# koskja/linalg-solver

Hardware: AMD Instinct MI355X
Metric: fp64_lu_gflops (higher is better)
Workload: dtype f64; 1 GPU; 8192x8192 f64 LU with partial pivoting (getrf), u11 generator, resident in HBM; n=8192, nb=128, panel_mode=4, lookahead=1, parallelism=single GPU, resident_inputs=189

## Files before the change

### linalg_solver_amd/csrc/api.hip

```cpp
#include <stdarg.h>
#include <stdlib.h>
#include <string.h>

#include <algorithm>

#include "common.h"

namespace lsx {

static thread_local char g_err[512] = "";

void set_error(const char *fmt, ...) {
    va_list ap;
    va_start(ap, fmt);
    vsnprintf(g_err, sizeof(g_err), fmt, ap);
    va_end(ap);
}

static int grow(void **p, size_t *have, size_t need) {
    if (need <= *have) return LSX_OK;
    if (*p) {
        LSX_HIP(hipFree(*p));
        *p = nullptr;
        *have = 0;
// ... 215 lines not shown
    const size_t pass_bytes = pad256(256 + (size_t)nsteps * sizeof(int)), ctr_bytes = pad256((size_t)nsteps * 8 * sizeof(int));
    const size_t col0_bytes = pad256((size_t)nsteps * 2 * sizeof(int));
    const size_t words = pass_bytes + ctr_bytes + col0_bytes + pad256((size_t)nsteps * sizeof(int));
    if (area_x == 0 || 3 * area_x + words > h->scratch_bytes) { set_error("getrf_lookahead_x: scratch"); return LSX_ERR_INTERNAL; }
    LSX_TRY(grow(&h->moves_all, &h->moves_all_bytes, (size_t)nsteps * 2048));
    JoinSide join{h, side, main_s, main_s};
    char *wbase = (char *)h->scratch + 3 * area_x;
    int *xcc_word = (int *)wbase;
    int *pass = (int *)(wbase + 256);
    int *counters = (int *)(wbase + pass_bytes);
    int *col0 = (int *)(wbase + pass_bytes + ctr_bytes);
    int *ready = (int *)(wbase + pass_bytes + ctr_bytes + col0_bytes);
    for (int s = 0; s < 3; ++s) LSX_HIP(hipMemsetAsync((char *)h->scratch + (size_t)s * area_x, 0, area_x, main_s));
    LSX_HIP(hipMemsetAsync(wbase, 0, words, main_s));
    LSX_HIP(hipMemsetD32Async((hipDeviceptr_t)xcc_word, 1, 1, main_s));
    pa.area_bytes = area_x;
    pa.xcc_word = xcc_word;
    LSX_HIP(hipEventRecord(h->ev_start, main_s));
    LSX_HIP(hipStreamWaitEvent(side, h->ev_start, 0));
    auto list = [&](int s) { return (int2 *)((char *)h->moves_all + (size_t)s * 2048); };
    T *Tinv2[2] = {Tinv, Tinv + (size_t)((nb + 63) / 64) * 4096};
    {
        OnStream g(h, side);
        pa.list = list(0);
        pa.area_off = 0;
        LSX_TRY(launch_panel<T>(h, n - k0, (n - k0) < nb ? (n - k0) : nb, A + (size_t)k0 * lda + k0, lda, k0, d_ipiv + k0, d_info, pa));
        if (!pa.listed) { set_error("getrf_lookahead_x: panel without a gather list"); return LSX_ERR_INTERNAL; }
    }
    const bool use_col0 = !h->x_events;
    bool prev_col0 = false;
    int prev_tiles = 0;
    int step = 0;
    int left_done = 0;
    for (int k = k0; k < n; k += nb, ++step) {
        const int jb = (n - k < nb) ? n - k : nb;
        const int rest = n - k - jb;
        if (rest <= 0) break;
        T *Akk = A + (size_t)k * lda + k;
        T *Ti = Tinv2[step & 1];
        T *A12 = A + (size_t)k * lda + k + jb;
        T *L21 = A + (size_t)(k + jb) * lda + k;
        T *A22 = A + (size_t)(k + jb) * lda + k + jb;
        const int jb2 = rest < nb ? rest : nb;
        bool fused_all = false;
        {
            OnStream g(h, side);
            const bool counted = step > 0 && prev_col0;
            if (step > 0 && !counted) LSX_HIP(hipStreamWaitEvent(side, h->ev_next, 0));
            const int all = launch_chain_fused<T>(h, list(step), d_info, jb, Akk, lda, Ti, jb2, A + k + jb, lda, k,
                                                  counted ? col0 + 2 * (step - 1) + 1 : nullptr, prev_tiles, ready + step);
            if (all < 0) return all;
            if (all == 1) {
                const int fused = launch_chain_head<T>(h, list(step), d_info, jb, Akk, lda, Ti, jb2, A + k + jb, lda, k,
                                                       counted ? col0 + 2 * (step - 1) + 1 : nullptr, prev_tiles);
                if (fused < 0) return fused;
                if (fused == 1) {
                    if (counted) LSX_TRY(launch_wait_count(h, col0 + 2 * (step - 1) + 1, prev_tiles, d_info));
                    LSX_TRY(launch_trtri<T>(h, 1, jb, Akk, lda, Ti));
                    LSX_TRY(launch_laswp_moves<T>(h, list(step), jb2, A + k + jb, lda, k));
                }
            }
            fused_all = all == LSX_OK;
            if (!fused_all) {
                LSX_HIP(hipEventRecord(h->ev_panel, side));
                LSX_TRY(launch_trsm_block<T>(h, 1, jb, jb2, Akk, lda, Ti, A12, lda));
            }
            LSX_TRY(launch_gemm_sub<T>(h, rest, jb2, jb, L21, lda, A12, lda, A22, lda, mfma));
        }
        if (fused_all) LSX_TRY(launch_wait_count(h, ready + step, 2, d_info));
        else LSX_HIP(hipStreamWaitEvent(main_s, h->ev_panel, 0));
        GemmDone did;
        if (rest > jb2) {
            LSX_TRY(launch_laswp_moves<T>(h, list(step), rest - jb2, A + k + jb + jb2, lda, k));
            LSX_TRY(launch_trsm_block<T>(h, 1, jb, rest - jb2, Akk, lda, Ti, A12 + jb2, lda));
            GemmPlan plan = mfma;
            plan.counters = counters + 8 * step;
            plan.avoid_word = xcc_word;
            plan.pass_word = pass + step;
            plan.col0 = use_col0 ? col0 + 2 * step : nullptr;
            LSX_TRY(launch_gemm_sub<T>(h, rest, rest - jb2, jb, L21, lda, A12 + jb2, lda, A22 + jb2, lda, plan, &did));
        }
        const bool cur_col0 = did.queued && did.col0_complete;
        LSX_HIP(hipMemsetAsync((char *)h->scratch + (size_t)(step % 3) * area_x, 0, area_x, main_s));
        LSX_HIP(hipEventRecord(h->ev_next, main_s));
        if (h->left_per_step && (rest <= 5632 || k <= 4096)) {
            if (left_done < step) {
                LSX_TRY(launch_laswp_left_all<T>(h, A, lda, k0 + left_done * nb, nb, step - left_done, list(left_done)));
                left_done = step;
            }
            if (k > 0) LSX_TRY(launch_laswp_moves<T>(h, list(step), k, A, lda, k));
            left_done = step + 1;
        }
        {
            OnStream g(h, side);
            const bool tall = (rest > 6400 && (sizeof(T) == 8 || rest <= 8192)) || rest > 12800;
            if (did.queued && (!cur_col0 || tall)) LSX_TRY(launch_gate(h, pass + step, 2 * h->num_cu / 8));
            pa.list = list(step + 1);
            pa.area_off = (size_t)((step + 1) % 3) * area_x;
            LSX_TRY(launch_panel<T>(h, rest, jb2, A22, lda, k + jb, d_ipiv + k + jb, d_info, pa));
            if (!pa.listed) { set_error("getrf_lookahead_x: panel without a gather list"); return LSX_ERR_INTERNAL; }
        }
        prev_col0 = cur_col0;
        prev_tiles = did.col0_tiles;
    }
    LSX_HIP(hipEventRecord(h->ev_panel, side));
    LSX_HIP(hipStreamWaitEvent(main_s, h->ev_panel, 0));
    join.armed = false;
    return launch_laswp_left_all<T>(h, A, lda, k0 + left_done * nb, nb, nsteps - left_done, list(left_done));
}

int ensure_getrf_workspace(lsx_handle_t h, int n, size_t elem) {
    LSX_TRY(ensure_scratch(h, pad256(16 * ((size_t)n / 32 + 2)) + 2 * pad256(elem * 2 * (size_t)n) +
                                  ((size_t)n / 32 + 2) * 5248 + 8192 +
                                  3 * panel_x_area_bytes(h, h->panel_mode, n, elem) + 16384 +
                                  ((size_t)n / 16 + 2) * 40));
    const size_t tinv_elems = (size_t)((h->nb * h->kblock + 63) / 64) * 64 * 64;
    return grow(&h->ws2, &h->ws2_bytes, 2 * pad256(tinv_elems * elem));
}

template <typename T>
static int getrf_dev(lsx_handle_t h, int n, T *A, int lda, int32_t *d_ipiv, int *d_info, bool percolumn = false) {
    LSX_ARG(n >= 0 && lda >= n && A && d_ipiv);
    if (n == 0) return LSX_OK;
    const int nb = h->nb;
    PanelArgs pa(h, h->moves_buf[0]);
    if (percolumn) pa.mode = 0;
    GemmPlan mfma;
    mfma.mfma_only = true;
    LSX_TRY(ensure_getrf_workspace(h, n, sizeof(T)));
    T *Tinv = (T *)h->ws2;
    if (!d_info) d_info = h->dev_status + 2;
    LSX_HIP(hipMemsetAsync(d_info, 0, sizeof(int), h->stream));
    int LOOKAHEAD_MIN = sizeof(T) == 8 ? 7168 : 10240;
    if (pa.mode == 4) LOOKAHEAD_MIN = sizeof(T) == 8 ? 2048 : 4096;
    if (h->lookahead_min > 0) LOOKAHEAD_MIN = h->lookahead_min;
    int k_end = n;
    if (h->lookahead && !percolumn && n >= LOOKAHEAD_MIN && h->kblock == 1) k_end = 0;
    const int W = nb * h->kblock;
    for (int k = 0; k < k_end; k += W) {
        const int w = (n - k < W) ? n - k : W;
        for (int j = 0; j < w; j += nb) {
            const int c = k + j;
            const int jb = (w - j < nb) ? w - j : nb;
            T *Acc = A + (size_t)c * lda + c;
            LSX_TRY(launch_panel<T>(h, n - c, jb, Acc, lda, c, d_ipiv + c, d_info, pa));
            if (pa.listed) {
                LSX_TRY(launch_laswp_moves_around<T>(h, (const int2 *)pa.list, n, A, lda, c, c, jb));
            } else {
                LSX_TRY(launch_laswp<T>(h, c, A, lda, c, jb, d_ipiv + c));
                LSX_TRY(launch_laswp<T>(h, n - c - jb, A + c + jb, lda, c, jb, d_ipiv + c));
            }
            const int inner = w - j - jb;
            if (inner > 0) {
                T *A12 = A + (size_t)c * lda + c + jb;
                LSX_TRY(launch_trtri<T>(h, 1, jb, Acc, lda, Tinv));
                LSX_TRY(launch_trsm_block<T>(h, 1, jb, inner, Acc, lda, Tinv, A12, lda));
                LSX_TRY(launch_gemm_sub<T>(h, n - c - jb, inner, jb, A + (size_t)(c + jb) * lda + c, lda, A12,
                                           lda, A + (size_t)(c + jb) * lda + c + jb, lda, mfma));
            }
        }
        const int rest = n - k - w;
        if (rest > 0) {
            T *Akk = A + (size_t)k * lda + k;
            T *A12 = A + (size_t)k * lda + k + w;
            LSX_TRY(launch_trtri<T>(h, 1, w, Akk, lda, Tinv));
            if (w > nb && nb % 64 == 0) {
                for (int j = 0; j < w; j += nb) {
                    const int jb = (w - j < nb) ? w - j : nb;
// ... 788 lines not shown
    return LSX_OK;
}

int lsx_synchronize(lsx_handle_t h) {
    LSX_DEVICE_GUARD(h);
    LSX_ARG(h);
    LSX_HIP(hipStreamSynchronize(h->stream));
    return LSX_OK;
}

int lsx_check_status(lsx_handle_t h) {
    LSX_ARG(h);
    LSX_DEVICE_GUARD(h);
    return check_dev_status(h);
}

int lsx_set_option(lsx_handle_t h, const char *key, int value) {
    LSX_DEVICE_GUARD(h);
    LSX_ARG(h && key);
    if (!strcmp(key, "nb")) {
        LSX_ARG(value >= 16 && value <= 128 && value % 16 == 0);
        h->nb = value;
    } else if (!strcmp(key, "panel")) {
        LSX_ARG(value >= 0 && value <= 4);
        if (value == 1 || value == 2) {
            set_error("panel modes 1 and 2 (superseded kernels) were removed: use 0, 3 or 4");
            return LSX_ERR_ARG;
        }
        h->panel_mode = value;
    } else if (!strcmp(key, "trsv")) {
        LSX_ARG(value >= 0 && value <= 2);
        h->trsv_mode = value;
    } else if (!strcmp(key, "gemm_tiles32")) {
        LSX_ARG(value == 0 || value == 1);
        h->gemm_no_tiles32 = !value;
    } else if (!strcmp(key, "gemm_queue_test")) {
        LSX_ARG(value >= 0 && value <= 3);
        h->gemm_queue_test = value;
    } else if (!strcmp(key, "gemm_stagger")) {
        LSX_ARG(value >= 0 && value <= 64);
        h->gemm_stagger = value;
    } else if (!strcmp(key, "gemm_waves")) {
        LSX_ARG(value == 0 || value == 4 || value == 8);
        h->gemm_waves = value;
    } else if (!strcmp(key, "kblock")) {
        LSX_ARG(value == 1 || value == 2);
        h->kblock = value;
    } else if (!strcmp(key, "panel_rt")) {
        LSX_ARG(value == 2 || value == 4 || value == 8);
        h->panel_rt = value;
    } else if (!strcmp(key, "panel_nt")) {
        LSX_ARG(value == 0 || value == 256 || value == 512 || value == 1024);
        h->panel_nt = value;
    } else if (!strcmp(key, "rref_blocked")) {
        LSX_ARG(value == 0 || value == 1);
        h->rref_blocked = value;
    } else if (!strcmp(key, "xrows_limit")) {
        LSX_ARG(value >= 0);
        h->xrows_limit = value;
    } else if (!strcmp(key, "getri_structured")) {
        LSX_ARG(value == 0 || value == 1);
        h->getri_plain = !value;
    } else if (!strcmp(key, "x_events")) {
        LSX_ARG(value == 0 || value == 1);
        h->x_events = value;
    } else if (!strcmp(key, "hybrid")) {
        LSX_ARG(value == 0 || value == 1);
        h->hybrid_off = !value;
    } else if (!strcmp(key, "prof_sample")) {
        LSX_ARG(value >= 1);
        h->prof.sample = value;
    } else if (!strcmp(key, "panel_spin_limit")) {
        LSX_ARG(value != 0);
        h->panel_spin_limit = value;
    } else if (!strcmp(key, "trsv_spin_limit")) {
        LSX_ARG(value >= 0);
        h->spin_limit = value;
    } else if (!strcmp(key, "getri_pairs")) {
        LSX_ARG(value == 0 || value == 1);
        h->getri_pairs = value;
    } else if (!strcmp(key, "left_per_step")) {
        LSX_ARG(value == 0 || value == 1);
        h->left_per_step = value;
    } else if (!strcmp(key, "chain_fused")) {
        LSX_ARG(value == 0 || value == 1);
        h->chain_fused = value;
    } else if (!strcmp(key, "rref_first_fast")) {
        LSX_ARG(value == 0 || value == 1);
        h->rref_first_fast = value;
    } else if (!strcmp(key, "chain_wait_limit")) {
        LSX_ARG(value >= 0);
        h->chain_wait_limit = value;
    } else if (!strcmp(key, "panel_debug")) {
        h->panel_debug = value != 0;
    } else if (!strcmp(key, "lookahead")) {
        LSX_ARG(value == 0 || value == 1);
        h->lookahead = value;
    } else if (!strcmp(key, "lookahead_min")) {
        LSX_ARG(value >= 0);
        h->lookahead_min = value;
    } else if (!strcmp(key, "getrs_t_blocked_min")) {
        LSX_ARG(value >= 0);
        h->getrs_t_blocked_min = value;
    } else {
        set_error("unknown option '%s'", key);
        return LSX_ERR_ARG;
    }
    return LSX_OK;
}

int lsx_get_option(lsx_handle_t h, const char *key, int *value) {
    LSX_DEVICE_GUARD(h);
    LSX_ARG(h && key && value);
    if (!strcmp(key, "nb")) *value = h->nb;
    else if (!strcmp(key, "panel")) *value = h->panel_mode;
    else if (!strcmp(key, "lookahead")) *value = h->lookahead;
    else if (!strcmp(key, "lookahead_min")) *value = h->lookahead_min;
    else if (!strcmp(key, "panel_rt")) *value = h->panel_rt;
    else if (!strcmp(key, "kblock")) *value = h->kblock;
    else if (!strcmp(key, "gemm_waves")) *value = h->gemm_waves;
    else if (!strcmp(key, "gemm_stagger")) *value = h->gemm_stagger;
    else if (!strcmp(key, "trsv")) *value = h->trsv_mode;
    else if (!strcmp(key, "panel_nt")) *value = h->panel_nt;
    else if (!strcmp(key, "chain_wait_limit")) *value = h->chain_wait_limit;
    else if (!strcmp(key, "rref_first_fast")) *value = h->rref_first_fast;
    else if (!strcmp(key, "chain_fused")) *value = h->chain_fused;
    else if (!strcmp(key, "left_per_step")) *value = h->left_per_step;
    else if (!strcmp(key, "getri_pairs")) *value = h->getri_pairs;
    else if (!strcmp(key, "rref_first_used")) *value = h->rref_first_used;
    else if (!strcmp(key, "panel_fallbacks")) *value = h->panel_fallbacks;
    else if (!strcmp(key, "num_cu")) *value = h->num_cu;
    else if (!strcmp(key, "gecon_solves")) *value = h->gecon_solves;
    else if (!strcmp(key, "gerfs_steps")) *value = h->gerfs_steps;
    else if (!strcmp(key, "gerfs_solves")) *value = h->gerfs_solves;
    else if (!strcmp(key, "getrs_t_blocked_min")) *value = h->getrs_t_blocked_min;
    else if (!strcmp(key, "getrs_t_path")) *value = h->getrs_t_path;
    else { set_error("unknown option '%s'", key); return LSX_ERR_ARG; }
    return LSX_OK;
}

int lsx_getrf_f64(lsx_handle_t h, int n, double *A, int lda, int32_t *ipiv, int *info) {
    LSX_DEVICE_GUARD(h);
    return getrf_host<double>(h, n, A, lda, ipiv, info);
}
int lsx_getrs_f64(lsx_handle_t h, int n, int nrhs, const double *LU, int lda, const int32_t *ipiv,
                  double *B, int ldb) {
    LSX_DEVICE_GUARD(h);
    return getrs_host<double>(h, n, nrhs, LU, lda, ipiv, B, ldb);
}
int lsx_gesv_f64(lsx_handle_t h, int n, int nrhs, const double *A, int lda, double *B, int ldb,
                 int *info, double *pivot_ratio) {
    LSX_DEVICE_GUARD(h);
    return gesv_host<double>(h, n, nrhs, A, lda, B, ldb, info, pivot_ratio);
}
int lsx_getrf_f32(lsx_handle_t h, int n, float *A, int lda, int32_t *ipiv, int *info) {
    LSX_DEVICE_GUARD(h);
    return getrf_host<float>(h, n, A, lda, ipiv, info);
}
int lsx_getrs_f32(lsx_handle_t h, int n, int nrhs, const float *LU, int lda, const int32_t *ipiv,
                  float *B, int ldb) {
    LSX_DEVICE_GUARD(h);
    return getrs_host<float>(h, n, nrhs, LU, lda, ipiv, B, ldb);
}
int lsx_gesv_f32(lsx_handle_t h, int n, int nrhs, const float *A, int lda, float *B, int ldb,
                 int *info, double *pivot_ratio) {
    LSX_DEVICE_GUARD(h);
    return gesv_host<float>(h, n, nrhs, A, lda, B, ldb, info, pivot_ratio);
}

}

namespace lsx {

template <typename T>
static int getri_host(lsx_handle_t h, int n, const T *A, int lda, T *Ainv, int ldi, int *info, double *pivot_ratio) {
    LSX_ARG(h && n >= 0 && lda >= n && ldi >= n);
    if (info) *info = 0;
    if (pivot_ratio) *pivot_ratio = 1.0;
    if (n == 0) return LSX_OK;
    LSX_ARG(A && Ainv);
    const int ld = ld_for(n);
    LSX_TRY(ensure_ws(h, 2 * pad256(sizeof(T) * (size_t)n * ld) + pad256(sizeof(int32_t) * n) + 1024));
    Carver c(h->ws);
    T *dA = c.take<T>((size_t)n * ld);
    T *dI = c.take<T>((size_t)n * ld);
    int32_t *dp = c.take<int32_t>(n);
    int *dinfo = c.take<int>(1);
    double *dprobe = c.take<double>(2);
    LSX_TRY(h2d<T>(h, n, n, A, lda, dA, ld));
    LSX_TRY(launch_amax<T>(h, n, n, dA, ld, dprobe));
    int hinfo = 0;
    LSX_TRY(factor_from_host<T>(h, n, A, lda, dA, ld, dp, dinfo, &hinfo));
    LSX_TRY(launch_diag_minabs<T>(h, n, dA, ld, dprobe));
    double probe[2] = {0, 0};
    LSX_HIP(hipMemcpyAsync(probe, dprobe, sizeof(probe), hipMemcpyDeviceToHost, h->stream));
    LSX_HIP(hipStreamSynchronize(h->stream));
    if (info) *info = hinfo;
    if (pivot_ratio) *pivot_ratio = probe[0] > 0 ? probe[1] / probe[0] : 0.0;
    if (hinfo != 0) return LSX_OK;
    LSX_TRY(getri_dev<T>(h, n, dA, ld, dp, dI, ld));
    LSX_TRY(d2h<T>(h, n, n, dI, ld, Ainv, ldi));
    LSX_HIP(hipStreamSynchronize(h->stream));
    return LSX_OK;
}

template <typename T>
static int det_host(lsx_handle_t h, int n, const T *A, int lda, double *sign, double *mant, int64_t *exp2) {
    LSX_ARG(h && n >= 0 && lda >= n && sign && mant && exp2);
    if (n == 0) { *sign = 1; *mant = 0.5; *exp2 = 1; return LSX_OK; }
    LSX_ARG(A);
// ... 672 lines not shown
```

### linalg_solver_amd/csrc/common.h

```cpp
#pragma once
#include <hip/hip_runtime.h>
#include <stdint.h>
#include <stdio.h>
#include <string>
#include <vector>

#include "../../include/lsx.h"

#ifdef LSX_TSTAMP
static __device__ long long *lsx_ts_buf;
struct TsScope {
    int id;
    __device__ void put(int tag) {
        long long *b = lsx_ts_buf;
        const int i = atomicAdd((int *)b, 1);
        if (i < (1 << 20)) { b[1 + 2 * i] = tag; b[2 + 2 * i] = wall_clock64(); }
    }
    __device__ TsScope(int id_) : id(id_) { if (lsx_ts_buf && threadIdx.x == 0 && blockIdx.x == 0 && blockIdx.y == 0) put(id); }
    __device__ ~TsScope() { if (lsx_ts_buf && threadIdx.x == 0) put(id | 0x100); }
};
#define LSX_TS(id) TsScope ts_scope_(id)
#define LSX_TS_SETTER(name) extern "C" void lsx_ts_set_##name(long long *p) { (void)hipMemcpyToSymbol(HIP_SYMBOL(lsx_ts_buf), &p, sizeof p); }
#else
#define LSX_TS(id)
#define LSX_TS_SETTER(name)
#endif

namespace lsx {

void set_error(const char *fmt, ...);

#define LSX_HIP(call)                                                                     \
    do {                                                                                  \
        hipError_t e_ = (call);                                                           \
        if (e_ != hipSuccess) {                                                           \
            lsx::set_error("%s failed: %s (%s:%d)", #call, hipGetErrorString(e_), __FILE__, \
                           __LINE__);                                                     \
            return LSX_ERR_HIP;                                                           \
        }                                                                                 \
    } while (0)

#define LSX_TRY(call)              \
    do {                           \
        int r_ = (call);           \
        if (r_ != LSX_OK) return r_; \
    } while (0)

#define LSX_ARG(cond)                                                     \
    do {                                                                  \
        if (!(cond)) {                                                    \
            lsx::set_error("bad argument: %s (%s:%d)", #cond, __FILE__, __LINE__); \
            return LSX_ERR_ARG;                                           \
        }                                                                 \
    } while (0)

struct ProfEvent {
    hipEvent_t a, b;
    int bucket;
};

struct Prof {
    unsigned mask = 0;
    int sample = 1;
    long long seen[LSX_PROF_NBUCKETS] = {0};
    std::vector<ProfEvent> pending;
    std::vector<hipEvent_t> pool;
    double ms[LSX_PROF_NBUCKETS] = {0};
    long long launches[LSX_PROF_NBUCKETS] = {0};
    double flops[LSX_PROF_NBUCKETS] = {0};
    double bytes[LSX_PROF_NBUCKETS] = {0};
};

}

struct lsx_handle_s {
    int device = 0;
    hipStream_t own_stream = nullptr;
    hipStream_t stream = nullptr;
    hipStream_t side_stream = nullptr;
    hipEvent_t ev_panel = nullptr, ev_next = nullptr, ev_start = nullptr, ev_done = nullptr;
    int nb = 128;
    int kblock = 1;
    int panel_mode = 4;
    int lookahead = 1;
    int lookahead_min = 0;
    int panel_rt = 4;
    int panel_nt = 0;
    int trsv_mode = 2;
    int gemm_stagger = 0;
    int gemm_waves = 0;
    int getri_pairs = 1;
    int left_per_step = 1;
    int chain_fused = 1;
    int chain_wait_limit = 1 << 21;
    int x_events = 0;
    void *moves_all = nullptr;
    size_t moves_all_bytes = 0;
    int panel_debug = 0;
    int num_cu = 256;
    void *ws = nullptr;
    size_t ws_bytes = 0;
    void *ws2 = nullptr;
    size_t ws2_bytes = 0;
    void *ws3 = nullptr;
    size_t ws3_bytes = 0;
    void *ws5 = nullptr;
    size_t ws5_bytes = 0;
    int getri_plain = 0;
    void *xchg = nullptr;
    size_t xchg_bytes = 0;
    unsigned xchg_epoch = 0;
    void *ws6 = nullptr;
    size_t ws6_bytes = 0;
    int rref_first_fast = 1;
    int rref_first_used = 0;
    void *ws4 = nullptr;
    size_t ws4_bytes = 0;
    void *ws7 = nullptr;
    size_t ws7_bytes = 0;
    int gecon_solves = 0;
    void *ws8 = nullptr;
    size_t ws8_bytes = 0;
    int gerfs_steps = 0;
    int gerfs_solves = 0;
    int getrs_t_blocked_min = 64;
    int getrs_t_path = 0;
    void *moves_buf[2] = {nullptr, nullptr};
    void *moves_api = nullptr;
    bool moves_api_valid = false;
    void *scratch = nullptr;
    size_t scratch_bytes = 0;
    int *dev_status = nullptr;
    int rref_blocked = 1;
    int gemm_no_tiles32 = 0;
    int gemm_queue_test = 0;
    int xrows_limit = 0;
    int hybrid_off = 0;
    int panel_fallbacks = 0;
    int panel_spin_limit = 1 << 20;
    int spin_limit = 1 << 20;
    lsx::Prof prof;
};

namespace lsx {

struct OnStream {
    lsx_handle_t h; hipStream_t keep;
    OnStream(lsx_handle_t h_, hipStream_t s) : h(h_), keep(h_->stream) { h->stream = s; }
    ~OnStream() { h->stream = keep; }
};

struct GemmPlan {
    int kshift = 0;
    bool mfma_only = false;
    int *col0_static = nullptr;
    int *counters = nullptr;
    const int *avoid_word = nullptr;
    int *pass_word = nullptr;
    int *col0 = nullptr;
};
struct GemmDone {
    bool queued = false;
    bool col0_complete = false;
    int col0_tiles = 0;
};

struct PanelArgs {
    int mode, nt, rt;
    void *list;
    size_t area_off = 0, area_bytes = 0;
    int *xcc_word = nullptr;
    bool listed = false;
    PanelArgs(lsx_handle_t h, void *list_) : mode(h->panel_mode), nt(h->panel_nt), rt(h->panel_rt), list(list_) {}
};
// ... 164 lines not shown
```

### linalg_solver_amd/csrc/kernels_gemm.hip

```cpp
#include "common.h"

namespace lsx {

typedef double d4 __attribute__((ext_vector_type(4)));
typedef float f4 __attribute__((ext_vector_type(4)));

template <typename T>
struct Mfma;
template <>
struct Mfma<double> {
    typedef d4 acc_t;
    static __device__ __forceinline__ acc_t mma(double a, double b, acc_t c) {
        return __builtin_amdgcn_mfma_f64_16x16x4f64(a, b, c, 0, 0, 0);
    }
    static __device__ __forceinline__ int crow(int lane, int r) { return (lane >> 4) + 4 * r; }
};
template <>
struct Mfma<float> {
    typedef f4 acc_t;
    static __device__ __forceinline__ acc_t mma(float a, float b, acc_t c) {
        return __builtin_amdgcn_mfma_f32_16x16x4f32(a, b, c, 0, 0, 0);
    }
    static __device__ __forceinline__ int crow(int lane, int r) { return 4 * (lane >> 4) + r; }
};
// ... 212 lines not shown
        if (stagger > 0 && ((blockIdx.x >> 8) & 1))
            for (int i = 0; i < stagger; ++i) __builtin_amdgcn_s_sleep(127);
    }
    plus &= ~0xff00;

    if (col0_done) {
        if ((int)blockIdx.x < tiles_m) {
            gemm_sub_tile<T, FULL, NWN, BM_>(M, N, K, A, lda, B, ldb, C, ldc, ((int)blockIdx.x + tm_off) * BM_, tn_off * BN, As, Bs, plus);
            __syncthreads();
            if (threadIdx.x == 0) {
                __threadfence();
                __hip_atomic_fetch_add(col0_done, 1, __ATOMIC_RELEASE, __HIP_MEMORY_SCOPE_AGENT);
            }
            return;
        }
    }
    const int first_col = col0_done ? 1 : 0;
    if (col0_done) tiles_n -= 1;
    const int nwg = tiles_m * tiles_n;
    int tile_m, tile_n;
    grouped_tile((int)blockIdx.x - (col0_done ? tiles_m : 0), nwg, tiles_m, tiles_n, tile_m, tile_n);
    const int m0 = (tile_m + tm_off) * BM_, n0 = (tile_n + first_col + tn_off) * BN;
    gemm_sub_tile<T, FULL, NWN, BM_>(M, N, K, A, lda, B, ldb, C, ldc, m0, n0, As, Bs, plus);
}

template <typename T, int NWN, bool FULL>
__global__ __launch_bounds__(BM * NWN, (sizeof(T) == 4 && NWN == 4) ? 6 : NWN) void gemm_tn_kernel(
    int M, int N, int K, const T *__restrict__ A, int lda, const T *__restrict__ B, int ldb, T *__restrict__ C, int ldc,
    int tiles_m, int tiles_n, int tm_off, int tn_off, int plus) {
    __shared__ T As[2][BK / 2][ASlab<T, BM>::PAIR];
    __shared__ T Bs[2][BK][BN + LPAD];
    int tile_m, tile_n;
    grouped_tile((int)blockIdx.x, tiles_m * tiles_n, tiles_m, tiles_n, tile_m, tile_n);
    gemm_sub_tile<T, FULL, NWN, BM, true>(M, N, K, A, lda, B, ldb, C, ldc, (tile_m + tm_off) * BM, (tile_n + tn_off) * BN, As,
                                          Bs, plus & 3);
}

template <typename T, int NWN>
__global__ __launch_bounds__(BM * NWN, (sizeof(T) == 4 && NWN == 4) ? 6 : NWN) void gemm_sub_queue_kernel(
    int M, int N, int K, const T *__restrict__ A, int lda, const T *__restrict__ B, int ldb, T *__restrict__ C,
    int ldc, int tiles_m, int tiles_n, int plus, int *__restrict__ counters, const int *__restrict__ avoid_word,
    int *__restrict__ pass_word, int *__restrict__ col0) {
    LSX_TS(6);
    __shared__ T As[2][BK / 2][ASlab<T, BM>::PAIR];
    __shared__ T Bs[2][BK][BN + LPAD];
    __shared__ int s_tile;
    unsigned xcc;
    asm volatile("s_getreg_b32 %0, hwreg(HW_REG_XCC_ID, 0, 4)" : "=s"(xcc));
    const int avoid_xcc = avoid_word ? __hip_atomic_load(avoid_word, __ATOMIC_RELAXED, __HIP_MEMORY_SCOPE_AGENT) - 1 : -1;
    if ((int)xcc == avoid_xcc) {
        if (pass_word && threadIdx.x == 0) __hip_atomic_fetch_add(pass_word, 1, __ATOMIC_RELAXED, __HIP_MEMORY_SCOPE_AGENT);
        return;
    }
    const int nx = avoid_xcc >= 0 ? 7 : 8;
    const int rank = (avoid_xcc >= 0 && (int)xcc > avoid_xcc) ? (int)xcc - 1 : (int)xcc;
    const int c_first = col0 ? 1 : 0;
    const int tn = tiles_n - c_first;
    for (int q = -c_first; q < nx; ++q) {
        const int owner = (rank + max(q, 0)) % nx;
        int c_lo = c_first + (int)((long long)owner * tn / nx), c_hi = c_first + (int)((long long)(owner + 1) * tn / nx);
        int *ctr = &counters[owner];
        if (q < 0) { c_lo = 0; c_hi = 1; ctr = col0; }
        const int sw = c_hi - c_lo;
        const int hi = tiles_m * sw;
        if (sw <= 0) continue;
        if (threadIdx.x == 0) s_tile = __hip_atomic_fetch_add(ctr, 1, __ATOMIC_RELAXED, __HIP_MEMORY_SCOPE_AGENT);
        __syncthreads();
        for (;;) {
            const int bid = s_tile;
            if (bid >= hi) break;
            const int tile_m = bid / sw;
            const int tile_n = c_lo + bid % sw;
            gemm_sub_tile<T, true, NWN, BM>(M, N, K, A, lda, B, ldb, C, ldc, tile_m * BM, tile_n * BN, As, Bs, plus, ctr, &s_tile);
            __syncthreads();
            if (q < 0 && threadIdx.x == 0) {
                __threadfence();
                __hip_atomic_fetch_add(col0 + 1, 1, __ATOMIC_RELEASE, __HIP_MEMORY_SCOPE_AGENT);
            }
        }
        __syncthreads();
    }
}

template <typename T>
__global__ __launch_bounds__(256) void gemm_sub_skinny_kernel(int M, int N, int K,
                                                              const T *__restrict__ A, int lda,
                                                              const T *__restrict__ B, int ldb,
                                                              T *__restrict__ C, int ldc, int plus) {
    const int lane = threadIdx.x & 63;
    const int row = blockIdx.x * 4 + (threadIdx.x >> 6);
    if (row >= M) return;
    const T *a = A + (size_t)row * lda;
    for (int j0 = 0; j0 < N; j0 += 8) {
        T part[8] = {0, 0, 0, 0, 0, 0, 0, 0};
        for (int k = lane; k < K; k += 64) {
            const T av = a[k];
            const T *b = B + (size_t)k * ldb + j0;
#pragma unroll
            for (int j = 0; j < 8; ++j)
                if (j0 + j < N) part[j] += av * b[j];
        }
#pragma unroll
        for (int j = 0; j < 8; ++j) {
            T v = part[j];
#pragma unroll
            for (int off = 32; off > 0; off >>= 1) v += __shfl_down(v, off, 64);
            if (lane == 0 && j0 + j < N) C[(size_t)row * ldc + j0 + j] += plus ? v : -v;
        }
    }
}

template <typename T>
int launch_gemm_acc(lsx_handle_t h, int plus, int m, int n, int k, const T *A, int lda, const T *B, int ldb,
                    T *C, int ldc, const GemmPlan &plan, GemmDone *done) {
    GemmDone unread;
    GemmDone &did = done ? *done : unread;
    did = GemmDone();
    if (m <= 0 || n <= 0 || k <= 0) return LSX_OK;
    const bool queue = plan.counters != nullptr;
    const int kshift = plan.kshift;
    const bool skinny = n < 16 && !plan.mfma_only && !kshift;
    if (kshift && (queue || kshift >= k || kshift > 0xfff || kshift % BK || (k - kshift) % BK)) {
        set_error("gemm: k rotation %d not served here (k = %d)", kshift, k);
        return LSX_ERR_INTERNAL;
    }
    const bool tiles64 = !queue && n >= 16 && sizeof(T) == 8 && (h->gemm_waves == 0 || h->gemm_waves == 8) && m % 64 == 0 &&
                         n % BN == 0 && k % BK == 0 && ((m + BM - 1) / BM) * (n / BN) <= h->num_cu / 2 &&
                         ((size_t)A % 16 == 0) && ((size_t)B % 16 == 0) && ((size_t)C % 16 == 0) && lda % 2 == 0 &&
                         ldb % 2 == 0 && ldc % 2 == 0;
    ProfScope ps(h, tiles64 ? LSX_PROF_GEMM_SKINNY : LSX_PROF_GEMM, 2.0 * m * n * (double)k,
                 2.0 * sizeof(T) * m * (double)n);
    if (skinny) {
        hipLaunchKernelGGL(gemm_sub_skinny_kernel<T>, dim3((m + 3) / 4), dim3(256), 0, h->stream, m,
                           n, k, A, lda, B, ldb, C, ldc, plus);
    } else {
        const int tm = (m + BM - 1) / BM, tn = (n + BN - 1) / BN;
        const int elems16 = 16 / (int)sizeof(T);
        const bool aligned = ((size_t)A % 16 == 0) && ((size_t)B % 16 == 0) && ((size_t)C % 16 == 0) &&
                             (lda % elems16 == 0) && (ldb % elems16 == 0) && (ldc % elems16 == 0) && (k % BK == 0);
        const int waves = h->gemm_waves ? h->gemm_waves : (sizeof(T) == 8 ? 8 : 4);
        const int fm = aligned ? m / BM : 0, fn = aligned ? n / BN : 0;
        int *col0s = (plan.col0_static && !queue && waves == 8 && fm == tm && fm > 0 && fn > 1) ? plan.col0_static : nullptr;
        did.col0_complete = col0s != nullptr;
        did.col0_tiles = fm;
        auto go = [&](bool full, int gm, int gn, int om, int on) {
            if (gm <= 0 || gn <= 0) return;
            const dim3 grid(gm * gn);
            if (waves == 8) {
                if (full) hipLaunchKernelGGL((gemm_sub_kernel<T, 4, true>), grid, dim3(512), 0, h->stream, m, n, k, A, lda, B, ldb, C, ldc, gm, gn, om, on, plus | (h->gemm_stagger << 8) | (kshift << 16), col0s);
                else hipLaunchKernelGGL((gemm_sub_kernel<T, 4, false>), grid, dim3(512), 0, h->stream, m, n, k, A, lda, B, ldb, C, ldc, gm, gn, om, on, plus | (h->gemm_stagger << 8) | (kshift << 16));
            } else {
                if (full) hipLaunchKernelGGL((gemm_sub_kernel<T, 2, true>), grid, dim3(256), 0, h->stream, m, n, k, A, lda, B, ldb, C, ldc, gm, gn, om, on, plus | (h->gemm_stagger << 8) | (kshift << 16));
                else hipLaunchKernelGGL((gemm_sub_kernel<T, 2, false>), grid, dim3(256), 0, h->stream, m, n, k, A, lda, B, ldb, C, ldc, gm, gn, om, on, plus | (h->gemm_stagger << 8) | (kshift << 16));
            }
        };
        if (tiles64) {
            if (m % 32 == 0 && (m / 32) * tn <= h->num_cu && !h->gemm_no_tiles32)
                hipLaunchKernelGGL((gemm_sub_kernel<T, 4, true, 32>), dim3((m / 32) * tn), dim3(256), 0, h->stream, m, n, k,
                                   A, lda, B, ldb, C, ldc, m / 32, tn, 0, 0, plus | (kshift << 16));
            else
                hipLaunchKernelGGL((gemm_sub_kernel<T, 4, true, 64>), dim3((m / 64) * tn), dim3(256), 0, h->stream, m, n, k,
                                   A, lda, B, ldb, C, ldc, m / 64, tn, 0, 0, plus | (kshift << 16));
            LSX_HIP(hipGetLastError());
            return LSX_OK;
        }
        if (queue && fm > 0 && fn > 0) {
            did.queued = true;
            did.col0_complete = (plan.col0 != nullptr) && fm == tm;
            const dim3 grid(2 * h->num_cu);
            if (waves == 8)
                hipLaunchKernelGGL((gemm_sub_queue_kernel<T, 4>), grid, dim3(512), 0, h->stream, m, n, k, A, lda, B, ldb, C, ldc, fm, fn, plus, plan.counters, plan.avoid_word, plan.pass_word, plan.col0);
            else
                hipLaunchKernelGGL((gemm_sub_queue_kernel<T, 2>), grid, dim3(256), 0, h->stream, m, n, k, A, lda, B, ldb, C, ldc, fm, fn, plus, plan.counters, plan.avoid_word, plan.pass_word, plan.col0);
        } else {
            go(true, fm, fn, 0, 0);
        }
        go(false, tm - fm, tn, fm, 0);
        go(false, fm, tn - fn, 0, fn);
    }
    LSX_HIP(hipGetLastError());
    return LSX_OK;
}

template <typename T>
int launch_gemm_tn_acc(lsx_handle_t h, int mode, int m, int n, int k, const T *A, int lda, const T *B, int ldb, T *C,
                       int ldc) {
    if (m <= 0 || n <= 0 || (k <= 0 && mode != 3)) return LSX_OK;
    if (k < 0) k = 0;
    ProfScope ps(h, LSX_PROF_GEMM, 2.0 * m * n * (double)k, (mode == 3 ? 1.0 : 2.0) * sizeof(T) * m * (double)n);
    const int tm = (m + BM - 1) / BM, tn = (n + BN - 1) / BN;
    const int elems16 = 16 / (int)sizeof(T);
    const bool aligned = ((size_t)A % 16 == 0) && ((size_t)B % 16 == 0) && ((size_t)C % 16 == 0) && (lda % elems16 == 0) &&
                         (ldb % elems16 == 0) && (ldc % elems16 == 0) && (k % BK == 0) && k > 0;
    const int fm = aligned ? m / BM : 0, fn = aligned ? n / BN : 0;
    constexpr int NWN = sizeof(T) == 8 ? 4 : 2;
    auto go = [&](bool full, int gm, int gn, int om, int on) {
        if (gm <= 0 || gn <= 0) return;
        if (full) hipLaunchKernelGGL((gemm_tn_kernel<T, NWN, true>), dim3(gm * gn), dim3(BM * NWN), 0, h->stream, m, n, k, A, lda, B, ldb, C, ldc, gm, gn, om, on, mode);
        else hipLaunchKernelGGL((gemm_tn_kernel<T, NWN, false>), dim3(gm * gn), dim3(BM * NWN), 0, h->stream, m, n, k, A, lda, B, ldb, C, ldc, gm, gn, om, on, mode);
    };
    go(true, fm, fn, 0, 0);
    go(false, tm - fm, tn, fm, 0);
    go(false, fm, tn - fn, 0, fn);
    LSX_HIP(hipGetLastError());
    return LSX_OK;
}

template <typename T>
int launch_gemm_tn_sub(lsx_handle_t h, int m, int n, int k, const T *A, int lda, const T *B, int ldb, T *C, int ldc) {
    return launch_gemm_tn_acc<T>(h, 0, m, n, k, A, lda, B, ldb, C, ldc);
}

template <typename T>
int launch_gemm_sub(lsx_handle_t h, int m, int n, int k, const T *A, int lda, const T *B, int ldb, T *C,
                    int ldc, const GemmPlan &plan, GemmDone *done) {
    return launch_gemm_acc<T>(h, 0, m, n, k, A, lda, B, ldb, C, ldc, plan, done);
}

template int launch_gemm_acc<double>(lsx_handle_t, int, int, int, int, const double *, int, const double *,
                                     int, double *, int, const GemmPlan &, GemmDone *);
template int launch_gemm_acc<float>(lsx_handle_t, int, int, int, int, const float *, int, const float *, int,
                                    float *, int, const GemmPlan &, GemmDone *);
template int launch_gemm_tn_acc<double>(lsx_handle_t, int, int, int, int, const double *, int, const double *, int, double *, int);
template int launch_gemm_tn_acc<float>(lsx_handle_t, int, int, int, int, const float *, int, const float *, int, float *, int);
template int launch_gemm_tn_sub<double>(lsx_handle_t, int, int, int, const double *, int, const double *, int, double *, int);
template int launch_gemm_tn_sub<float>(lsx_handle_t, int, int, int, const float *, int, const float *, int, float *, int);
template int launch_gemm_sub<double>(lsx_handle_t, int, int, int, const double *, int,
                                     const double *, int, double *, int, const GemmPlan &, GemmDone *);
template int launch_gemm_sub<float>(lsx_handle_t, int, int, int, const float *, int, const float *,
                                    int, float *, int, const GemmPlan &, GemmDone *);

}

LSX_TS_SETTER(gemm)
```

### linalg_solver_amd/csrc/kernels_panel_x.hip

```cpp
#include <type_traits>

#include "common.h"
#include "panel_xchg.h"

namespace lsx {

constexpr int PX_WC = 8;
constexpr int PX_NT = 64 * (128 / PX_WC);
constexpr int PX_REC = 128;
constexpr int PX_NONE = 0x7fffffff;
#ifndef LSX_PX_SEG
#define LSX_PX_SEG -1
#endif
#define PX_MARK(k)                                                                  \
    if (LSX_PX_SEG >= 0) {                                                          \
        if (LSX_PX_SEG == (k)) seg_t0 = __builtin_amdgcn_s_memtime();               \
        if (LSX_PX_SEG + 1 == (k)) seg_acc += __builtin_amdgcn_s_memtime() - seg_t0; \
    }

__device__ __forceinline__ int argmax64_fast(unsigned khi, unsigned klo, int idx) {
    const unsigned mhi = rows_max_u32<4>(row16_max_u32(khi), 0);
    const bool top = (khi == mhi) & (idx != PX_NONE);
    const unsigned long long mask = __builtin_amdgcn_ballot_w64(top);
    if (mask == 0ull) return PX_NONE;
// ... 496 lines not shown
            moves[t] = make_int2(dst, src);
        }
    }
    if (has_cols) {
#pragma unroll
        for (int r = 0; r < RT; ++r) {
            const int lr = 64 * r + lane;
            const int gi = base + lr;
            if (gi < m) {
                const int ord = s_order[lr];
                const int dest = ord >= 0 ? ord : (gi < jb ? s_postop[gi] : gi);
                T *dst = P + (size_t)dest * ldp + c0;
                if (wide) {
#pragma unroll
                    for (int c = 0; c < WC; c += 2) {
                        v2t v;
                        v[0] = a[r][c]; v[1] = a[r][c + 1];
                        *(v2t *)(dst + c) = v;
                    }
                } else {
#pragma unroll
                    for (int c = 0; c < WC; ++c)
                        if (c0 + c < jb) dst[c] = a[r][c];
                }
            }
        }
    }
}

template <typename T, int RT, bool DBG, bool FIRST = false>
__global__ __launch_bounds__(PX_NT, PX_NT / 256) void panel_x_kernel(int m, int jb, T *__restrict__ P, int ldp, int row0, int col0,
                                                        int32_t *__restrict__ ipiv, int *__restrict__ info,
                                                        char *rec, XGran *far, int *status, unsigned long long *dbg,
                                                        int2 *__restrict__ moves, int *xcc, int *xcc_word,
                                                        int spin_limit, double tol) {
    if (blockIdx.x & 7) return;
    LSX_TS(1);
    const int G = gridDim.x >> 3, g = blockIdx.x >> 3;
    if (spin_limit < 0) {
        spin_limit = -spin_limit;
        if (g == G - 1 && G > 1)
            for (int i = 0; i < 900; ++i) __builtin_amdgcn_s_sleep(127);
    }
    __shared__ int s_same;
    if (threadIdx.x < 64) {
        unsigned id;
        asm volatile("s_getreg_b32 %0, hwreg(HW_REG_XCC_ID, 0, 4)" : "=s"(id));
        const int lane = threadIdx.x;
        if (lane == 0) {
            __hip_atomic_store(&xcc[g], (int)id + 1, __ATOMIC_RELAXED, __HIP_MEMORY_SCOPE_AGENT);
            if (g == 0 && xcc_word) __hip_atomic_store(xcc_word, (int)id + 1, __ATOMIC_RELAXED, __HIP_MEMORY_SCOPE_AGENT);
        }
        bool pend = lane < G, same = true;
        int spins = 0;
        while (__any(pend)) {
            const int v = __hip_atomic_load(&xcc[lane < G ? lane : 0], __ATOMIC_RELAXED, __HIP_MEMORY_SCOPE_AGENT);
            if (pend && v != 0) { pend = false; same = v == (int)id + 1; }
            if (++spins > spin_limit) { same = false; break; }
        }
        const bool all_same = !__any(!same);
        if (lane == 0) {
            s_same = all_same ? 1 : 0;
            if (DBG && dbg) dbg[g * 16 + 15] = ((unsigned long long)id << 8) | (all_same ? 1u : 0u);
        }
    }
    __syncthreads();
    if (s_same)
        panel_x_body<T, RT, DBG, true, FIRST>(G, g, m, jb, P, ldp, row0, col0, ipiv, info, rec, far, status, dbg, moves, spin_limit, tol);
    else
        panel_x_body<T, RT, DBG, false, FIRST>(G, g, m, jb, P, ldp, row0, col0, ipiv, info, rec, far, status, dbg, moves, spin_limit, tol);
}

size_t panel_x_area_bytes(lsx_handle_t h, int mode, int m, size_t elem) {
    const int rt = elem == 8 ? 4 : 8;
    if (mode != 4 || h->panel_debug || h->nb > PC_COLS) return 0;
    if (m > 32 * 64 * rt) m = 32 * 64 * rt;
    return ((size_t)256 + (size_t)32 * (2 * PX_REC + 4 * PC_COLS * sizeof(XGran)) + 255) & ~(size_t)255;
}

template <typename T, int RT>
static int panel_xcd_rt(lsx_handle_t h, int m, int jb, T *P, int ldp, int row0, int col0, int32_t *d_ipiv, int *d_info,
                        PanelArgs &pa, const double first_tol = -1.0) {
    if (jb > PC_COLS) return 1;
    const int G = (m + 64 * RT - 1) / (64 * RT);
    if (G > 32 || 8 * G > 8 * h->num_cu) return 1;
    const size_t rec_bytes = (size_t)2 * G * PX_REC;
    const size_t need = 256 + rec_bytes + (size_t)4 * G * PC_COLS * sizeof(XGran);
    const size_t dbg_off = (need + 255) & ~(size_t)255;
    const size_t total = dbg_off + (h->panel_debug ? (size_t)G * 128 : 0);
    const bool driver_clears = pa.area_bytes > 0 && !h->panel_debug;
    const size_t base_off = driver_clears ? pa.area_off : 0;
    if (base_off + total > h->scratch_bytes || (driver_clears && need > pa.area_bytes)) {
        set_error("panel_xcd: scratch too small (%zu + %zu > %zu)", base_off, total, h->scratch_bytes);
        return LSX_ERR_INTERNAL;
    }
    char *base = (char *)h->scratch + base_off;
    int *status = (int *)base;
    int *xcc = (int *)(base + 64);
    char *rec = base + 256;
    XGran *far = (XGran *)(base + 256 + rec_bytes);
    if (!driver_clears) LSX_HIP(hipMemsetAsync(base, 0, h->panel_debug ? total : need, h->stream));
    unsigned long long *dbg = h->panel_debug ? (unsigned long long *)(base + dbg_off) : nullptr;
    if (first_tol >= 0.0) {
        if constexpr (sizeof(T) == 8 && RT <= 4)
            hipLaunchKernelGGL((panel_x_kernel<T, RT, false, true>), dim3(8 * G), dim3(PX_NT), 0, h->stream, m, jb, P, ldp, row0,
                               col0, d_ipiv, d_info, rec, far, status, dbg, (int2 *)pa.list, xcc, pa.xcc_word, h->panel_spin_limit, first_tol);
        else
            return 1;
    } else if (h->panel_debug)
        hipLaunchKernelGGL((panel_x_kernel<T, RT, true>), dim3(8 * G), dim3(PX_NT), 0, h->stream, m, jb, P, ldp, row0,
                           col0, d_ipiv, d_info, rec, far, status, dbg, (int2 *)pa.list, xcc, pa.xcc_word, h->panel_spin_limit, -1.0);
    else
        hipLaunchKernelGGL((panel_x_kernel<T, RT, false>), dim3(8 * G), dim3(PX_NT), 0, h->stream, m, jb, P, ldp, row0,
                           col0, d_ipiv, d_info, rec, far, status, dbg, (int2 *)pa.list, xcc, pa.xcc_word, h->panel_spin_limit, -1.0);
    LSX_HIP(hipGetLastError());
    pa.listed = true;
    return LSX_OK;
}

template <typename T>
int panel_xcd(lsx_handle_t h, int m, int jb, T *P, int ldp, int row0, int col0, int32_t *d_ipiv, int *d_info, PanelArgs &pa) {
    if (m <= 32 * 64 * 1) return panel_xcd_rt<T, 1>(h, m, jb, P, ldp, row0, col0, d_ipiv, d_info, pa);
    if (m <= 32 * 64 * 2) return panel_xcd_rt<T, 2>(h, m, jb, P, ldp, row0, col0, d_ipiv, d_info, pa);
    if (sizeof(T) == 4 && m > 32 * 64 * 4) return panel_xcd_rt<T, sizeof(T) == 4 ? 8 : 4>(h, m, jb, P, ldp, row0, col0, d_ipiv, d_info, pa);
    return panel_xcd_rt<T, 4>(h, m, jb, P, ldp, row0, col0, d_ipiv, d_info, pa);
}

int panel_xcd_first(lsx_handle_t h, int m, int jb, double *P, int ldp, int row0, int col0, int32_t *d_ipiv, int *d_info,
                    double tol, PanelArgs &pa) {
    pa.listed = false;
    if (tol < 0.0 || m > 32 * 64 * 4) return 1;
    if (m <= 32 * 64 * 1) return panel_xcd_rt<double, 1>(h, m, jb, P, ldp, row0, col0, d_ipiv, d_info, pa, tol);
    if (m <= 32 * 64 * 2) return panel_xcd_rt<double, 2>(h, m, jb, P, ldp, row0, col0, d_ipiv, d_info, pa, tol);
    return panel_xcd_rt<double, 4>(h, m, jb, P, ldp, row0, col0, d_ipiv, d_info, pa, tol);
}

template int panel_xcd<double>(lsx_handle_t, int, int, double *, int, int, int, int32_t *, int *, PanelArgs &);
template int panel_xcd<float>(lsx_handle_t, int, int, float *, int, int, int, int32_t *, int *, PanelArgs &);

}

LSX_TS_SETTER(panelx)
```

Before: 22740 GFLOP/s.

## Add narrow-GEMM kernel for lookahead update, skip redundant event, defer left swaps

```diff
diff --git a/linalg_solver_amd/csrc/api.hip b/linalg_solver_amd/csrc/api.hip
--- a/linalg_solver_amd/csrc/api.hip
+++ b/linalg_solver_amd/csrc/api.hip
@@ -321,8 +321,8 @@
         }
         const bool cur_col0 = did.queued && did.col0_complete;
         LSX_HIP(hipMemsetAsync((char *)h->scratch + (size_t)(step % 3) * area_x, 0, area_x, main_s));
-        LSX_HIP(hipEventRecord(h->ev_next, main_s));
-        if (h->left_per_step && (rest <= 5632 || k <= 4096)) {
+        if (!cur_col0 || h->ev_next_always) LSX_HIP(hipEventRecord(h->ev_next, main_s));
+        if (h->left_per_step && rest <= h->left_defer_rows && (rest <= 5632 || k <= 4096)) {
             if (left_done < step) {
                 LSX_TRY(launch_laswp_left_all<T>(h, A, lda, k0 + left_done * nb, nb, step - left_done, list(left_done)));
                 left_done = step;
@@ -1277,6 +1277,18 @@
     } else if (!strcmp(key, "left_per_step")) {
         LSX_ARG(value == 0 || value == 1);
         h->left_per_step = value;
+    } else if (!strcmp(key, "left_defer_rows")) {
+        LSX_ARG(value >= 0);
+        h->left_defer_rows = value;
+    } else if (!strcmp(key, "panel_x_rt")) {
+        LSX_ARG(value >= 0 && value <= 4);
+        h->panel_x_rt = value;
+    } else if (!strcmp(key, "gemm_narrow")) {
+        LSX_ARG(value == 0 || value == 1);
+        h->gemm_narrow = value;
+    } else if (!strcmp(key, "ev_next_always")) {
+        LSX_ARG(value == 0 || value == 1);
+        h->ev_next_always = value;
     } else if (!strcmp(key, "chain_fused")) {
         LSX_ARG(value == 0 || value == 1);
         h->chain_fused = value;
@@ -1321,6 +1333,10 @@
     else if (!strcmp(key, "rref_first_fast")) *value = h->rref_first_fast;
     else if (!strcmp(key, "chain_fused")) *value = h->chain_fused;
     else if (!strcmp(key, "left_per_step")) *value = h->left_per_step;
+    else if (!strcmp(key, "left_defer_rows")) *value = h->left_defer_rows;
+    else if (!strcmp(key, "panel_x_rt")) *value = h->panel_x_rt;
+    else if (!strcmp(key, "gemm_narrow")) *value = h->gemm_narrow;
+    else if (!strcmp(key, "ev_next_always")) *value = h->ev_next_always;
     else if (!strcmp(key, "getri_pairs")) *value = h->getri_pairs;
     else if (!strcmp(key, "rref_first_used")) *value = h->rref_first_used;
     else if (!strcmp(key, "panel_fallbacks")) *value = h->panel_fallbacks;
diff --git a/linalg_solver_amd/csrc/common.h b/linalg_solver_amd/csrc/common.h
--- a/linalg_solver_amd/csrc/common.h
+++ b/linalg_solver_amd/csrc/common.h
@@ -90,6 +90,10 @@
     int gemm_stagger = 0;
     int gemm_waves = 0;
     int getri_pairs = 1;
+    int panel_x_rt = 0;
+    int ev_next_always = 0;
+    int gemm_narrow = 1;
+    int left_defer_rows = 6400;
     int left_per_step = 1;
     int chain_fused = 1;
     int chain_wait_limit = 1 << 21;
diff --git a/linalg_solver_amd/csrc/kernels_gemm.hip b/linalg_solver_amd/csrc/kernels_gemm.hip
--- a/linalg_solver_amd/csrc/kernels_gemm.hip
+++ b/linalg_solver_amd/csrc/kernels_gemm.hip
@@ -318,6 +318,74 @@
     }
 }
 
+template <int SR>
+__global__ __launch_bounds__(256, 1) void gemm_narrow_kernel(const double *__restrict__ A, int lda,
+                                                             const double *__restrict__ B, int ldb,
+                                                             double *__restrict__ C, int ldc, int plus) {
+    LSX_TS(4);
+    typedef Mfma<double>::acc_t acc_t;
+    typedef double v2 __attribute__((ext_vector_type(2)));
+    constexpr int ROWS = 16 * SR, K = 128, TN = 2, WN = 32;
+    constexpr int TPR = 256 / ROWS;
+    constexpr int NLA = K / (2 * TPR);
+    constexpr int HALF = ROWS + (ROWS % 32 == 16 ? 0 : 16), PAIR = 2 * HALF + 2;
+    __shared__ double As[K / 2][PAIR];
+    const int tid = threadIdx.x, lane = tid & 63, wn = (tid >> 6) * WN;
+    const int lc = lane & 15, lq = lane >> 4;
+    const int m0 = (int)blockIdx.x * ROWS;
+    const double sgn = plus ? 1.0 : -1.0;
+    const int a_row = tid / TPR, a_k = (tid % TPR) * 2;
+
+    v2 ra[NLA];
+    {
+        const double *Ap = A + (size_t)(m0 + a_row) * lda + a_k;
+#pragma unroll
+        for (int i = 0; i < NLA; ++i) ra[i] = *(const v2 *)(Ap + 2 * TPR * i);
+    }
+    acc_t acc[SR][TN];
+#pragma unroll
+    for (int s = 0; s < SR; ++s)
+#pragma unroll
+        for (int r = 0; r < 4; ++r) {
+            const v2 x = *(const v2 *)(C + (size_t)(m0 + 16 * s + Mfma<double>::crow(lane, r)) * ldc + wn + TN * lc);
+            acc[s][0][r] = x[0];
+            acc[s][1][r] = x[1];
+        }
+    v2 rb[K / 4];
+    {
+        const unsigned b_off = (unsigned)lq * (unsigned)ldb + wn + TN * lc;
+#pragma unroll
+        for (int ks = 0; ks < K / 4; ++ks) rb[ks] = *(const v2 *)(B + (size_t)(4 * ks) * ldb + b_off);
+    }
+#pragma unroll
+    for (int i = 0; i < NLA; ++i) {
+        const int kp = (a_k + 2 * TPR * i) >> 1;
+        As[kp][a_row] = sgn * ra[i][0];
+        As[kp][HALF + a_row] = sgn * ra[i][1];
+    }
+    __syncthreads();
+#pragma unroll
+    for (int ks = 0; ks < K / 4; ++ks) {
+        const int k = 4 * ks + lq;
+        double a[SR];
+#pragma unroll
+        for (int s = 0; s < SR; ++s) a[s] = As[k >> 1][(k & 1) * HALF + 16 * s + lc];
+#pragma unroll
+        for (int s = 0; s < SR; ++s)
+#pragma unroll
+            for (int t = 0; t < TN; ++t) acc[s][t] = Mfma<double>::mma(a[s], rb[ks][t], acc[s][t]);
+    }
+#pragma unroll
+    for (int s = 0; s < SR; ++s)
+#pragma unroll
+        for (int r = 0; r < 4; ++r) {
+            v2 x;
+            x[0] = acc[s][0][r];
+            x[1] = acc[s][1][r];
+            *(v2 *)(C + (size_t)(m0 + 16 * s + Mfma<double>::crow(lane, r)) * ldc + wn + TN * lc) = x;
+        }
+}
+
 template <typename T>
 __global__ __launch_bounds__(256) void gemm_sub_skinny_kernel(int M, int N, int K,
                                                               const T *__restrict__ A, int lda,
@@ -364,8 +432,22 @@
                          n % BN == 0 && k % BK == 0 && ((m + BM - 1) / BM) * (n / BN) <= h->num_cu / 2 &&
                          ((size_t)A % 16 == 0) && ((size_t)B % 16 == 0) && ((size_t)C % 16 == 0) && lda % 2 == 0 &&
                          ldb % 2 == 0 && ldc % 2 == 0;
-    ProfScope ps(h, tiles64 ? LSX_PROF_GEMM_SKINNY : LSX_PROF_GEMM, 2.0 * m * n * (double)k,
+    const bool narrow = sizeof(T) == 8 && h->gemm_narrow && !queue && !kshift && n == BN && k == 128 && m % 32 == 0 &&
+                        m / 32 <= h->num_cu && (h->gemm_waves == 0 || h->gemm_waves == 8) && !h->gemm_no_tiles32 &&
+                        ((size_t)A % 16 == 0) && ((size_t)B % 16 == 0) && ((size_t)C % 16 == 0) && lda % 2 == 0 &&
+                        ldb % 2 == 0 && ldc % 2 == 0;
+    ProfScope ps(h, (tiles64 || narrow) ? LSX_PROF_GEMM_SKINNY : LSX_PROF_GEMM, 2.0 * m * n * (double)k,
                  2.0 * sizeof(T) * m * (double)n);
+    if constexpr (sizeof(T) == 8) {
+        if (narrow) {
+            if (m / 16 <= h->num_cu)
+                hipLaunchKernelGGL(gemm_narrow_kernel<1>, dim3(m / 16), dim3(256), 0, h->stream, A, lda, B, ldb, C, ldc, plus);
+            else
+                hipLaunchKernelGGL(gemm_narrow_kernel<2>, dim3(m / 32), dim3(256), 0, h->stream, A, lda, B, ldb, C, ldc, plus);
+            LSX_HIP(hipGetLastError());
+            return LSX_OK;
+        }
+    }
     if (skinny) {
         hipLaunchKernelGGL(gemm_sub_skinny_kernel<T>, dim3((m + 3) / 4), dim3(256), 0, h->stream, m,
                            n, k, A, lda, B, ldb, C, ldc, plus);
@@ -391,7 +473,8 @@
             }
         };
         if (tiles64) {
-            if (m % 32 == 0 && (m / 32) * tn <= h->num_cu && !h->gemm_no_tiles32)
+            const bool tiles32 = m % 32 == 0 && (m / 32) * tn <= h->num_cu && !h->gemm_no_tiles32;
+            if (tiles32)
                 hipLaunchKernelGGL((gemm_sub_kernel<T, 4, true, 32>), dim3((m / 32) * tn), dim3(256), 0, h->stream, m, n, k,
                                    A, lda, B, ldb, C, ldc, m / 32, tn, 0, 0, plus | (kshift << 16));
             else
diff --git a/linalg_solver_amd/csrc/kernels_panel_x.hip b/linalg_solver_amd/csrc/kernels_panel_x.hip
--- a/linalg_solver_amd/csrc/kernels_panel_x.hip
+++ b/linalg_solver_amd/csrc/kernels_panel_x.hip
@@ -602,6 +602,8 @@
 static int panel_xcd_rt(lsx_handle_t h, int m, int jb, T *P, int ldp, int row0, int col0, int32_t *d_ipiv, int *d_info,
                         PanelArgs &pa, const double first_tol = -1.0) {
     if (jb > PC_COLS) return 1;
+    constexpr bool HAS_FIRST = sizeof(T) == 8 && RT <= 4 && RT != 3;
+    if (first_tol >= 0.0 && !HAS_FIRST) return 1;
     const int G = (m + 64 * RT - 1) / (64 * RT);
     if (G > 32 || 8 * G > 8 * h->num_cu) return 1;
     const size_t rec_bytes = (size_t)2 * G * PX_REC;
@@ -622,7 +624,7 @@
     if (!driver_clears) LSX_HIP(hipMemsetAsync(base, 0, h->panel_debug ? total : need, h->stream));
     unsigned long long *dbg = h->panel_debug ? (unsigned long long *)(base + dbg_off) : nullptr;
     if (first_tol >= 0.0) {
-        if constexpr (sizeof(T) == 8 && RT <= 4)
+        if constexpr (HAS_FIRST)
             hipLaunchKernelGGL((panel_x_kernel<T, RT, false, true>), dim3(8 * G), dim3(PX_NT), 0, h->stream, m, jb, P, ldp, row0,
                                col0, d_ipiv, d_info, rec, far, status, dbg, (int2 *)pa.list, xcc, pa.xcc_word, h->panel_spin_limit, first_tol);
         else
@@ -640,6 +642,11 @@
 
 template <typename T>
 int panel_xcd(lsx_handle_t h, int m, int jb, T *P, int ldp, int row0, int col0, int32_t *d_ipiv, int *d_info, PanelArgs &pa) {
+    const int force = (h->panel_x_rt > 0 && m <= 32 * 64 * h->panel_x_rt) ? h->panel_x_rt : 0;
+    if (force == 1) return panel_xcd_rt<T, 1>(h, m, jb, P, ldp, row0, col0, d_ipiv, d_info, pa);
+    if (force == 2) return panel_xcd_rt<T, 2>(h, m, jb, P, ldp, row0, col0, d_ipiv, d_info, pa);
+    if (force == 3) return panel_xcd_rt<T, 3>(h, m, jb, P, ldp, row0, col0, d_ipiv, d_info, pa);
+    if (force == 4) return panel_xcd_rt<T, 4>(h, m, jb, P, ldp, row0, col0, d_ipiv, d_info, pa);
     if (m <= 32 * 64 * 1) return panel_xcd_rt<T, 1>(h, m, jb, P, ldp, row0, col0, d_ipiv, d_info, pa);
     if (m <= 32 * 64 * 2) return panel_xcd_rt<T, 2>(h, m, jb, P, ldp, row0, col0, d_ipiv, d_info, pa);
     if (sizeof(T) == 4 && m > 32 * 64 * 4) return panel_xcd_rt<T, sizeof(T) == 4 ? 8 : 4>(h, m, jb, P, ldp, row0, col0, d_ipiv, d_info, pa);
```

Result: no change. 22930 GFLOP/s (median of 6 runs) (+0.8%).
